# jianfch/stable-ts

Measured on AMD Instinct MI355X. Metric: real-time factor (audio-sec/wall-sec) large-v3 word_timestamps=True, higher is better.
Workload: dtype f16; 1 GPU; large-v3 (random-init, weight recipe BENCH_WEIGHTS = the parity-pinned recipe of tests/test_gpu_f16_depth.py), 10 min synthetic 16 kHz audio per GPU, word_timestamps=True, beam_size=5, 112 decode steps/window, window-parallel batch 20, default regrouping inside the timed pass; mode=transcribe, windows_per_gpu=20, segments=125, words=1670, parallelism=dp1 (windows sharded, no data-path collective)

## Files before the change

include/swx.h:

```cpp
#ifndef SWX_H
#define SWX_H
#include <stdint.h>
#include <stddef.h>

#ifdef __cplusplus
extern "C" {
#endif

#define SWX_F32 0
#define SWX_F16 1

#define SWX_N_SAMPLES 480000
#define SWX_N_FRAMES 3000
#define SWX_N_FFT 400
#define SWX_HOP 160

typedef struct swx_dims {
    int32_t n_mels, n_audio_ctx, n_audio_state, n_audio_head, n_audio_layer;
    int32_t n_vocab, n_text_ctx, n_text_state, n_text_head, n_text_layer;
} swx_dims;

typedef struct swx_model swx_model;

const char *swx_strerror(int code);
// ... 63 lines not shown

size_t swx_qcap_bytes(const swx_model *m, int max_n);
int swx_score_q(swx_model *m, const int32_t *d_tokens, const int32_t *h_n_tok, int max_n, int n_sot, int eot,
                const void *d_xkv, float *d_token_probs, void *d_q, void *stream);
size_t swx_heads_scratch_bytes(const swx_model *m, int max_n);
int swx_heads_dynamic(swx_model *m, const void *d_q, int max_n, int row0, int n_rows, const void *d_xkv, int n_frames,
                      float qk_scale, int count, const double *d_peaks, float *d_qk_sel, int ld_f, void *d_scratch,
                      size_t scratch_bytes, void *stream);
int swx_heads_new(swx_model *m, const void *d_q, int max_n, int n_tok, int row0, int n_out, const void *d_xkv, int n_frames,
                  float qk_scale, int medfilt_width, int topk, float w_colnorm, float w_rownorm, float w_coverage,
                  float *d_neg_matrix, int ld_f, void *d_scratch, size_t scratch_bytes, void *stream);
int swx_weighted_sum(const float *const *h_xs, const float *h_coef, int n_in, float *d_out, int64_t n, void *stream);

size_t swx_qcap_batch_bytes(const swx_model *m, int W, int max_n);
int swx_score_q_batch(swx_model *m, const int32_t *d_tokens, const int32_t *h_n_tok, int W, int max_n, int n_sot, int eot,
                      const void *d_xkv, int xkv_W, float *d_token_probs, void *d_q, void *stream);
size_t swx_heads_batch_scratch_bytes(const swx_model *m, int W, int max_n, int count);
int swx_heads_dynamic_batch(swx_model *m, const void *d_q, int W, int max_n, int n_sot, const int32_t *h_n_tok,
                            const int32_t *h_n_frames, const void *d_xkv, int xkv_W, float qk_scale, int medfilt_width, int count,
                            const double *d_peaks, float *d_neg_matrix, int ld_f, void *d_scratch, size_t scratch_bytes,
                            void *stream);
int swx_heads_new_batch(swx_model *m, const void *d_q, int W, int max_n, int n_sot, const int32_t *h_n_tok,
                        const int32_t *h_n_frames, const void *d_xkv, int xkv_W, float qk_scale, int medfilt_width, int topk,
                        float w_colnorm, float w_rownorm, float w_coverage, float *d_neg_matrix, int ld_f, void *d_scratch,
                        size_t scratch_bytes, void *stream);

int swx_forward_logits(swx_model *m, const int32_t *d_tokens, const int32_t *h_n_tok, int W, int max_n,
                       const void *d_xkv, float *d_logits, void *stream);

int swx_forward_token_ranks(swx_model *m, const int32_t *d_tokens, const int32_t *h_n_tok, int W, int max_n, int n_vocab_used,
                            const void *d_xkv, float *d_prob, int32_t *d_rank, void *stream);

int swx_forward_next_token(swx_model *m, const int32_t *d_tokens, const int32_t *h_n_tok, int W, int max_n, int eot,
                           const int32_t *d_suppress, int n_suppress, const int32_t *d_target,
                           const void *d_xkv, int32_t *d_top , float *d_prob , void *stream);

int swx_detect_language(swx_model *m, const void *d_xkv, int W, int sot, const int32_t *d_lang_tokens, int n_lang,
                        float *d_probs, int32_t *d_best, void *stream);

size_t swx_align_weights_scratch_bytes(int W, int H, int N);
int swx_align_weights(const float *d_qk, int W, int H, int N, int ld_f, const int32_t *h_n_frames, float qk_scale,
                      int medfilt_width, float *d_neg_matrix, void *d_scratch, size_t scratch_bytes, void *stream);

int swx_median_filter(const float *d_x, int64_t rows, int n, int width, float *d_out, void *stream);

int swx_loudness_probe(const float *d_pcm, int64_t pcm_stride, const int32_t *d_nk, const int32_t *d_idx, int n_idx, int W,
                       float *d_out, void *d_scratch, size_t scratch_bytes, void *stream);
size_t swx_loudness_probe_scratch_bytes(int W);

int swx_pcm_edit(const float *d_clean, float *d_probe, int64_t stride, int n_rows, const int32_t *d_ops,
                 const int32_t *d_row_start, int n_ops, void *stream);

typedef struct swx_gate_cfg {
    int32_t n_fft;
    int32_t n_mean;
    float   thresh, slope, prop_decrease;
    int32_t n_grad_freq, n_grad_time;
} swx_gate_cfg;
size_t swx_spectral_gate_scratch_bytes(int rows, const swx_gate_cfg *cfg);
int swx_spectral_gate(const float *d_pcm, int64_t pcm_stride, int rows, int64_t n, const swx_gate_cfg *cfg, float *d_out,
                      int64_t out_stride, void *d_scratch, size_t scratch_bytes, void *stream);
int swx_test_spectral_gate_block(int frames_per_block);

typedef struct swx_flac_info {
    int32_t sample_rate, channels, bits_per_sample, min_block, max_block;
    int64_t total_samples;
    uint8_t md5[16];
} swx_flac_info;
int swx_flac_probe(const uint8_t *h_data, size_t n_bytes, swx_flac_info *info);
int64_t swx_flac_decode(const uint8_t *h_data, size_t n_bytes, int32_t *h_out, int64_t capacity_frames, swx_flac_info *info);

size_t swx_dtw_workspace_bytes(int W, int ld_n, int ld_m);
int swx_dtw(const float *d_x, int W, int ld_n, int ld_m, const int32_t *d_N, const int32_t *d_M,
            int32_t *d_text_idx, int32_t *d_time_idx, int32_t *d_len, void *d_trace_ws, void *stream);

int swx_prof_enable(int on);
int swx_debug_flags(int flags);
int swx_prof_collect(double *out, int n_classes);
int swx_graph_stats(const swx_model *m, int64_t *out);

int swx_test_gemm(int dtype, const void *d_a, int64_t lda, const void *d_w, const float *d_bias, const void *d_res,
                  void *d_c, int64_t ldc, int M, int N, int K, int epilogue, int force_kernel, void *stream);
int swx_test_gemm_plan(int M, int N, int K, int epilogue, int force_kernel, int flags);
int swx_test_dec_gemm(const void *d_a, int64_t lda, const void *d_w, const float *d_gamma, const float *d_beta,
                      const float *d_bias, void *d_c, int64_t ldc, void *d_x, void *d_kcache, void *d_vcache,
                      const int32_t *d_pos0, int n_ctx, int d, int M, int N, int K, int epilogue, void *d_scratch,
                      size_t scratch_bytes, void *stream);
int swx_test_layernorm(int dtype, const void *d_x, const float *d_g, const float *d_b, void *d_y, int rows, int d,
                       void *stream);
int swx_test_attention(int dtype, const void *d_q, int64_t ldq, const void *d_k, const void *d_v, int64_t ldkv,
                       void *d_o, int64_t ldo, int B, int H, int nq, int nk, int force_kernel, int vt_kp, void *stream);

int swx_test_gemm_layout(int dtype, const void *d_a, int64_t lda, const void *d_w, int64_t ldw, const float *d_bias, const void *d_res,
                         const float *d_resf, int res_mod, void *d_c, int64_t ldc, void *d_c2, void *d_p, int64_t p_bs, int p_nkpad,
                         int p_vcol0, int vt_s, int vt_kp, int64_t vt_bs, int vt_zero_pad, int M, int N, int K, int epilogue,
                         int force_kernel, void *stream);
int swx_test_xkv_pack(const void *d_k, const void *d_vt, void *d_packed, int B, int H, int nk, int ldk, int vt_kp, int64_t batch_stride,
                      void *stream);
int swx_test_attention_packed(const void *d_q, int64_t ldq, const void *d_k, const void *d_v, int64_t ldkv, int64_t k_bs, int64_t v_bs,
                              const void *d_packed, void *d_o, int64_t ldo, int B, int H, int nq, int nk, int vt_kp, int force_kernel,
                              const void *d_x, int64_t ldx, int fq_rows, const void *d_wq, const float *d_gamma, const float *d_beta,
                              const float *d_bias, void *d_scratch, size_t scratch_bytes, void *stream);
int swx_test_xattn_plan(int B, int H, int nq, int nk, int vt_kp, int has_packed, int has_fq, int force_kernel, int flags);

int swx_test_self_attn_step(const void *d_q, void *d_kcache, void *d_vcache, const int32_t *d_anc, const int32_t *d_pos0,
                            int R, int H, int n_ctx, int d, int variant, void *d_o, void *stream);

int swx_test_self_attn_multi(const void *d_q, void *d_kcache, void *d_vcache, int R, int H, int n_new, int n_ctx, int d, int mq,
                             void *d_o, void *stream);

int swx_test_self_attn_general(int dtype, const void *d_qkv, int64_t ldqkv, void *d_kcache, void *d_vcache, const int32_t *d_anc,
                               const int32_t *d_pos0, int R, int H, int n_new, int n_ctx, int d, int row_mul, int skip_append,
                               int pos0_all_zero, void *d_o, void *stream);
int swx_test_kcache_index(int k_chunked, int n_ctx, int d, int pos, int h, int chunk);
int swx_test_kcache_relayout(const void *h_src, void *h_dst, int64_t rows, int n_ctx, int d, int elem_bytes, int to_chunked);
int swx_test_dec_gemm_kl(const void *d_a, int64_t lda, const void *d_w, const float *d_gamma, const float *d_beta,
                         const float *d_bias, void *d_c, int64_t ldc, void *d_x, void *d_kcache, void *d_vcache,
                         const int32_t *d_pos0, int n_ctx, int d, int M, int N, int K, int epilogue, int rps, int k_chunked,
                         void *d_scratch, size_t scratch_bytes, void *stream);
int swx_test_self_attn_step_kl(const void *d_q, void *d_kcache, void *d_vcache, const int32_t *d_anc, const int32_t *d_pos0,
                               int R, int H, int n_ctx, int d, int variant, int k_chunked, void *d_o, void *stream);
int swx_test_self_attn_multi_kl(const void *d_q, void *d_kcache, void *d_vcache, int R, int H, int n_new, int n_ctx, int d, int mq,
                                int k_chunked, void *d_o, void *stream);
int swx_test_self_attn_general_kl(int dtype, const void *d_qkv, int64_t ldqkv, void *d_kcache, void *d_vcache, const int32_t *d_anc,
                                  const int32_t *d_pos0, int R, int H, int n_new, int n_ctx, int d, int row_mul, int skip_append,
                                  int pos0_all_zero, int step_variant, int k_chunked, void *d_o, void *stream);
int swx_test_self_attn_plan(int dtype, int R, int H, int n_new, int n_ctx, int row_mul, int skip_append, int step_cached, int pos_bound,
                            int pos0_all_zero, int has_anc, int flags);
int swx_test_dec_plan(int M, int N, int K, int epilogue, int flags);
int swx_test_heads_layout(const swx_model *m, int W, int max_n, int count, int64_t *out);

int swx_test_lane_xor(const uint32_t *d_in, uint32_t *d_out, int n_waves, void *stream);

int swx_test_next_token_reduce(const float *d_logits, int64_t ld, int W, int eot, const int32_t *d_suppress, int n_suppress,
                               const int32_t *d_target, int32_t *d_top, float *d_prob, void *stream);

int swx_test_gelu_pair(uint64_t *d_out, void *stream);

size_t swx_test_decode_script_ws_bytes(const swx_decode_cfg *cfg, int n_vocab, int n_ctx);
int swx_test_decode_script(const swx_decode_cfg *cfg, int n_vocab, int n_ctx, const int32_t *d_init_tokens,
                           const int32_t *d_suppress, const uint8_t *d_ts_mask, const float *d_prefill_logits,
                           const float *d_script, int n_script, int32_t *d_tokens_out, int32_t *d_lens_out, float *d_sumlp_out,
                           float *d_nospeech, int32_t *d_anc_out, int32_t *d_pos0_out, void *d_ws, size_t ws_bytes, void *stream);

int swx_test_sampler_words(uint64_t seed, int64_t row_uid, int step, int id0, int n, uint32_t *d_words, float *d_variates, void *stream);
int swx_test_sampler_buckets(int k0, int n, float *d_variates, void *stream);

#ifdef __cplusplus
}
#endif
#endif
```

stable_ts_amd/_lib.py:

```python
import ctypes
import os
from ctypes import POINTER, Structure, c_char_p, c_float, c_int, c_int32, c_int64, c_size_t, c_uint64, c_void_p

_HERE = os.path.dirname(os.path.abspath(__file__))
LIB_PATH = os.path.join(_HERE, "libswx.so")

SWX_F32 = 0
SWX_F16 = 1


class SwxError(RuntimeError):
    pass


class swx_dims(Structure):
    _fields_ = [(n, c_int32) for n in ("n_mels", "n_audio_ctx", "n_audio_state", "n_audio_head", "n_audio_layer",
                                       "n_vocab", "n_text_ctx", "n_text_state", "n_text_head", "n_text_layer")]


class swx_flac_info(Structure):
    _fields_ = [("sample_rate", c_int32), ("channels", c_int32), ("bits_per_sample", c_int32), ("min_block", c_int32),
                ("max_block", c_int32), ("total_samples", c_int64), ("md5", ctypes.c_uint8 * 16)]


# ... 11 lines not shown
        ("no_speech", c_int32), ("blank_token", c_int32), ("n_suppress", c_int32), ("min_tokens", c_int32),
        ("seed", c_uint64), ("window_uid", POINTER(c_int32)), ("noise", c_void_p),
        ("sample_begins", POINTER(c_int32)), ("sot_indices", POINTER(c_int32)),
    ]


SYMBOLS = {
    "swx_strerror": (c_char_p, [c_int]),
    "swx_version": (c_int, []),
    "swx_model_create": (c_int, [POINTER(swx_dims), c_int, POINTER(c_void_p)]),
    "swx_model_destroy": (None, [c_void_p]),
    "swx_weights_bytes": (c_size_t, [c_void_p]),
    "swx_bind_weights": (c_int, [c_void_p, c_void_p, c_size_t]),
    "swx_share_weights": (c_int, [c_void_p, c_void_p]),
    "swx_load_tensor": (c_int, [c_void_p, c_char_p, c_void_p, c_int64, c_void_p]),
    "swx_weights_complete": (c_int, [c_void_p]),
    "swx_missing_tensor": (c_int, [c_void_p, c_int, c_char_p, c_int]),
    "swx_weights_mark_loaded": (c_int, [c_void_p]),
    "swx_weights_finalize": (c_int, [c_void_p, c_void_p]),
    "swx_set_alignment_heads": (c_int, [c_void_p, POINTER(c_int32), c_int]),
    "swx_num_alignment_heads": (c_int, [c_void_p]),
    "swx_workspace_bytes": (c_size_t, [c_void_p, c_int, c_int]),
    "swx_bind_workspace": (c_int, [c_void_p, c_void_p, c_size_t, c_int, c_int]),
    "swx_log_mel": (c_int, [c_void_p, c_void_p, c_int, c_void_p, c_int, c_void_p]),
    "swx_log_mel_ragged": (c_int, [c_void_p, c_void_p, c_void_p, c_void_p, c_int, c_void_p, c_int, c_void_p]),
    "swx_log_mel_ragged_grouped": (c_int, [c_void_p, c_void_p, c_void_p, c_void_p, c_int, c_void_p, c_int, c_void_p]),
    "swx_encode": (c_int, [c_void_p, c_void_p, c_int, c_void_p, c_void_p]),
    "swx_cross_kv_bytes": (c_size_t, [c_void_p, c_int]),
    "swx_cross_kv": (c_int, [c_void_p, c_void_p, c_int, c_void_p, c_void_p]),
    "swx_decode": (c_int, [c_void_p, POINTER(swx_decode_cfg), c_void_p, c_void_p, c_void_p, c_void_p, c_void_p,
                           c_void_p, c_void_p, c_void_p, c_void_p]),
    "swx_decode_gout": (c_int, [POINTER(swx_decode_cfg)]),
    "swx_score": (c_int, [c_void_p, c_void_p, POINTER(c_int32), c_int, c_int, c_int, c_int, POINTER(c_int32), c_float,
                          c_int, c_void_p, c_void_p, c_void_p, c_void_p]),
    "swx_score_qk": (c_int, [c_void_p, c_void_p, POINTER(c_int32), c_int, c_int, c_int, c_int, c_int, c_int, c_void_p,
                             c_void_p, c_void_p, c_void_p]),
    "swx_qcap_bytes": (c_size_t, [c_void_p, c_int]),
    "swx_score_q": (c_int, [c_void_p, c_void_p, POINTER(c_int32), c_int, c_int, c_int, c_void_p, c_void_p, c_void_p, c_void_p]),
    "swx_heads_scratch_bytes": (c_size_t, [c_void_p, c_int]),
    "swx_heads_dynamic": (c_int, [c_void_p, c_void_p, c_int, c_int, c_int, c_void_p, c_int, c_float, c_int, c_void_p, c_void_p,
                                  c_int, c_void_p, c_size_t, c_void_p]),
    "swx_heads_new": (c_int, [c_void_p, c_void_p, c_int, c_int, c_int, c_int, c_void_p, c_int, c_float, c_int, c_int, c_float,
                              c_float, c_float, c_void_p, c_int, c_void_p, c_size_t, c_void_p]),
    "swx_weighted_sum": (c_int, [c_void_p, c_void_p, c_int, c_void_p, c_int64, c_void_p]),
    "swx_qcap_batch_bytes": (c_size_t, [c_void_p, c_int, c_int]),
    "swx_score_q_batch": (c_int, [c_void_p, c_void_p, POINTER(c_int32), c_int, c_int, c_int, c_int, c_void_p, c_int, c_void_p,
                                  c_void_p, c_void_p]),
    "swx_heads_batch_scratch_bytes": (c_size_t, [c_void_p, c_int, c_int, c_int]),
    "swx_heads_dynamic_batch": (c_int, [c_void_p, c_void_p, c_int, c_int, c_int, POINTER(c_int32), POINTER(c_int32), c_void_p, c_int,
                                        c_float, c_int, c_int, c_void_p, c_void_p, c_int, c_void_p, c_size_t, c_void_p]),
    "swx_heads_new_batch": (c_int, [c_void_p, c_void_p, c_int, c_int, c_int, POINTER(c_int32), POINTER(c_int32), c_void_p, c_int,
                                    c_float, c_int, c_int, c_float, c_float, c_float, c_void_p, c_int, c_void_p, c_size_t, c_void_p]),
    "swx_forward_logits": (c_int, [c_void_p, c_void_p, POINTER(c_int32), c_int, c_int, c_void_p, c_void_p, c_void_p]),
    "swx_forward_token_ranks": (c_int, [c_void_p, c_void_p, POINTER(c_int32), c_int, c_int, c_int, c_void_p, c_void_p, c_void_p,
                                        c_void_p]),
    "swx_forward_next_token": (c_int, [c_void_p, c_void_p, POINTER(c_int32), c_int, c_int, c_int, c_void_p, c_int, c_void_p,
                                       c_void_p, c_void_p, c_void_p, c_void_p]),
    "swx_test_next_token_reduce": (c_int, [c_void_p, c_int64, c_int, c_int, c_void_p, c_int, c_void_p, c_void_p, c_void_p,
                                           c_void_p]),
    "swx_detect_language": (c_int, [c_void_p, c_void_p, c_int, c_int, c_void_p, c_int, c_void_p, c_void_p, c_void_p]),
    "swx_align_weights_scratch_bytes":(c_size_t, [c_int, c_int, c_int]),
    "swx_align_weights": (c_int, [c_void_p, c_int, c_int, c_int, c_int, POINTER(c_int32), c_float, c_int, c_void_p,
                                  c_void_p, c_size_t, c_void_p]),
    "swx_median_filter": (c_int, [c_void_p, c_int64, c_int, c_int, c_void_p, c_void_p]),
    "swx_loudness_probe": (c_int, [c_void_p, c_int64, c_void_p, c_void_p, c_int, c_int, c_void_p, c_void_p, c_size_t, c_void_p]),
    "swx_loudness_probe_scratch_bytes": (c_size_t, [c_int]),
    "swx_pcm_edit": (c_int, [c_void_p, c_void_p, c_int64, c_int, c_void_p, c_void_p, c_int, c_void_p]),
    "swx_spectral_gate_scratch_bytes": (c_size_t, [c_int, POINTER(swx_gate_cfg)]),
    "swx_spectral_gate": (c_int, [c_void_p, c_int64, c_int, c_int64, POINTER(swx_gate_cfg), c_void_p, c_int64, c_void_p, c_size_t,
                                  c_void_p]),
    "swx_test_spectral_gate_block": (c_int, [c_int]),
    "swx_flac_probe": (c_int, [c_void_p, c_size_t, POINTER(swx_flac_info)]),
    "swx_flac_decode": (c_int64, [c_void_p, c_size_t, c_void_p, c_int64, POINTER(swx_flac_info)]),
    "swx_dtw_workspace_bytes": (c_size_t, [c_int, c_int, c_int]),
    "swx_dtw": (c_int, [c_void_p, c_int, c_int, c_int, c_void_p, c_void_p, c_void_p, c_void_p, c_void_p, c_void_p,
                        c_void_p]),
    "swx_prof_enable": (c_int, [c_int]),
    "swx_debug_flags": (c_int, [c_int]),
    "swx_prof_collect": (c_int, [POINTER(ctypes.c_double), c_int]),
    "swx_graph_stats": (c_int, [c_void_p, POINTER(c_int64)]),
    "swx_test_gemm": (c_int, [c_int, c_void_p, c_int64, c_void_p, c_void_p, c_void_p, c_void_p, c_int64, c_int, c_int,
                              c_int, c_int, c_int, c_void_p]),
    "swx_test_gemm_plan": (c_int, [c_int, c_int, c_int, c_int, c_int, c_int]),
    "swx_test_dec_gemm": (c_int, [c_void_p, c_int64, c_void_p, c_void_p, c_void_p, c_void_p, c_void_p, c_int64, c_void_p,
                                  c_void_p, c_void_p, c_void_p, c_int, c_int, c_int, c_int, c_int, c_int, c_void_p, c_size_t,
                                  c_void_p]),
    "swx_test_self_attn_step": (c_int, [c_void_p, c_void_p, c_void_p, c_void_p, c_void_p, c_int, c_int, c_int, c_int, c_int, c_void_p,
                                        c_void_p]),
    "swx_test_self_attn_multi": (c_int, [c_void_p, c_void_p, c_void_p, c_int, c_int, c_int, c_int, c_int, c_int, c_void_p, c_void_p]),
    "swx_test_self_attn_general": (c_int, [c_int, c_void_p, c_int64, c_void_p, c_void_p, c_void_p, c_void_p, c_int, c_int, c_int, c_int,
                                           c_int, c_int, c_int, c_int, c_void_p, c_void_p]),
    "swx_test_kcache_index": (c_int, [c_int] * 6),
    "swx_test_kcache_relayout": (c_int, [c_void_p, c_void_p, c_int64, c_int, c_int, c_int, c_int]),
    "swx_test_dec_gemm_kl": (c_int, [c_void_p, c_int64, c_void_p, c_void_p, c_void_p, c_void_p, c_void_p, c_int64, c_void_p,
                                     c_void_p, c_void_p, c_void_p, c_int, c_int, c_int, c_int, c_int, c_int, c_int, c_int, c_void_p,
                                     c_size_t, c_void_p]),
    "swx_test_self_attn_step_kl": (c_int, [c_void_p, c_void_p, c_void_p, c_void_p, c_void_p, c_int, c_int, c_int, c_int, c_int, c_int,
                                           c_void_p, c_void_p]),
    "swx_test_self_attn_multi_kl": (c_int, [c_void_p, c_void_p, c_void_p, c_int, c_int, c_int, c_int, c_int, c_int, c_int, c_void_p,
                                            c_void_p]),
    "swx_test_self_attn_general_kl": (c_int, [c_int, c_void_p, c_int64, c_void_p, c_void_p, c_void_p, c_void_p, c_int, c_int, c_int,
                                              c_int, c_int, c_int, c_int, c_int, c_int, c_int, c_void_p, c_void_p]),
    "swx_test_self_attn_plan": (c_int, [c_int] * 12),
    "swx_test_dec_plan": (c_int, [c_int, c_int, c_int, c_int, c_int]),
    "swx_test_heads_layout": (c_int, [c_void_p, c_int, c_int, c_int, POINTER(c_int64)]),
    "swx_test_gelu_pair": (c_int, [c_void_p, c_void_p]),
    "swx_test_decode_script_ws_bytes": (c_size_t, [POINTER(swx_decode_cfg), c_int, c_int]),
    "swx_test_decode_script": (c_int, [POINTER(swx_decode_cfg), c_int, c_int, c_void_p, c_void_p, c_void_p, c_void_p, c_void_p,
                                       c_int, c_void_p, c_void_p, c_void_p, c_void_p, c_void_p, c_void_p, c_void_p, c_size_t,
                                       c_void_p]),
    "swx_test_sampler_words": (c_int, [c_uint64, c_int64, c_int, c_int, c_int, c_void_p, c_void_p, c_void_p]),
    "swx_test_sampler_buckets": (c_int, [c_int, c_int, c_void_p, c_void_p]),
    "swx_test_lane_xor": (c_int, [c_void_p, c_void_p, c_int, c_void_p]),
    "swx_test_layernorm": (c_int, [c_int, c_void_p, c_void_p, c_void_p, c_void_p, c_int, c_int, c_void_p]),
    "swx_test_attention": (c_int, [c_int, c_void_p, c_int64, c_void_p, c_void_p, c_int64, c_void_p, c_int64, c_int,
                                   c_int, c_int, c_int, c_int, c_int, c_void_p]),
    "swx_test_gemm_layout": (c_int, [c_int, c_void_p, c_int64, c_void_p, c_int64, c_void_p, c_void_p, c_void_p, c_int, c_void_p,
                                     c_int64, c_void_p, c_void_p, c_int64, c_int, c_int, c_int, c_int, c_int64, c_int, c_int, c_int,
                                     c_int, c_int, c_int, c_void_p]),
    "swx_test_xkv_pack": (c_int, [c_void_p, c_void_p, c_void_p, c_int, c_int, c_int, c_int, c_int, c_int64, c_void_p]),
    "swx_test_attention_packed": (c_int, [c_void_p, c_int64, c_void_p, c_void_p, c_int64, c_int64, c_int64, c_void_p, c_void_p,
                                          c_int64, c_int, c_int, c_int, c_int, c_int, c_int, c_void_p, c_int64, c_int, c_void_p,
                                          c_void_p, c_void_p, c_void_p, c_void_p, c_size_t, c_void_p]),
    "swx_test_xattn_plan": (c_int, [c_int] * 9),
}

_lib = None


def load(build_if_missing: bool = False) -> ctypes.CDLL:
    global _lib
    if _lib is not None:
        return _lib
    if not os.path.exists(LIB_PATH):
        if build_if_missing:
            from .build import build
            build(verbose=False)
        else:
            raise SwxError(f"{LIB_PATH} not found: build it with `python -m stable_ts_amd.build` "
                           f"(hipcc --offload-arch=gfx950). There is no CPU fallback.")
    lib = ctypes.CDLL(LIB_PATH)
    for name, (res, args) in SYMBOLS.items():
        fn = getattr(lib, name)
        fn.restype = res
        fn.argtypes = args
    _lib = lib
    return lib


def check(code: int, what: str = "") -> int:
    if code < 0:
        msg = load().swx_strerror(code).decode()
        raise SwxError(f"{what or 'libswx'} failed: {msg} ({code})")
    return code


def require_gpu():
    import torch
    if not torch.cuda.is_available():
        raise SwxError("stable_ts_amd needs a ROCm GPU (MI355X / gfx950); no CPU path exists in this package")
```

stable_ts_amd/csrc/swx_gemm.hip:

```cpp
#include <cstdlib>
#include <type_traits>
#include <array>
#include <vector>
#include <cstdio>
#include "swx_common.h"
#include "swx_kernels.h"

namespace {

template <typename T>
__device__ __forceinline__ void epilogue_store(const GemmArgs &g, int row, int col, float v)
{
    if (row >= g.M || col >= g.N) return;
    if (g.epi & EPI_BIAS) v += g.bias[col];
    if (g.epi & EPI_GELU) v = gelu_erf(v);
    if (g.epi & EPI_RESF32MOD) v += g.Rf[(size_t)(row % g.res_mod) * g.N + col];
    if (g.epi & EPI_RES) v += to_f32<T>(((const T *)g.R)[(size_t)row * g.ldr + col]);
    if (g.epi & EPI_STORE_VT) {
        const int w = row / g.vt_s, sidx = row - w * g.vt_s;
        ((T *)g.C)[(size_t)w * g.vt_bs + (size_t)col * g.vt_kp + sidx] = from_f32<T>(v);
    } else if (g.epi & EPI_CBATCH) {
        const int w = row / g.vt_s, sidx = row - w * g.vt_s;
        ((T *)g.C)[(size_t)w * g.vt_bs + (size_t)sidx * g.ldc + col] = from_f32<T>(v);
    } else if (g.epi & EPI_OUT_F32) ((float *)g.C)[(size_t)row * g.ldc + col] = v;
// ... 907 lines not shown
    const f16x8 zero8 = (f16x8)(f16)0;

    f16x8 wf[NKS_MAX];
#pragma unroll
    for (int ks = 0; ks < NKS_MAX; ++ks) {
        const f16x8 v = *(const f16x8 *)(wp + (ks < nks ? ks : nks - 1) * 32);
        wf[ks] = (nok && ks < nks) ? v : zero8;
    }

    f32x4 acc[MT];
#pragma unroll
    for (int t = 0; t < MT; ++t) acc[t] = (f32x4){0.f, 0.f, 0.f, 0.f};
    const f16 *ap[MT];
    bool aok[MT];
#pragma unroll
    for (int t = 0; t < MT; ++t) {
        const int m = t * 16 + fr;
        aok[t] = m < g.M;
        ap[t] = A + (size_t)(aok[t] ? m : 0) * g.lda + kb + fk;
    }
    f16x8 af[2][MT];
#pragma unroll
    for (int t = 0; t < MT; ++t) { const f16x8 v = *(const f16x8 *)(ap[t]); af[0][t] = aok[t] ? v : zero8; }
#pragma unroll
    for (int ks = 0; ks < NKS_MAX; ++ks) {
        if (ks < nks) {
            if (ks + 1 < nks) {
#pragma unroll
                for (int t = 0; t < MT; ++t) { const f16x8 v = *(const f16x8 *)(ap[t] + (ks + 1) * 32); af[(ks + 1) & 1][t] = aok[t] ? v : zero8; }
            }
#pragma unroll
            for (int t = 0; t < MT; ++t) acc[t] = __builtin_amdgcn_mfma_f32_16x16x32_f16(af[ks & 1][t], wf[ks], acc[t], 0, 0, 0);
        }
    }

    if (wave > 0) {
#pragma unroll
        for (int t = 0; t < MT; ++t) red[wave - 1][t][lane] = acc[t];
    }
    __syncthreads();
    if (wave == 0) {
        const int col = n0 + (lane & 15), row_l = (lane >> 4) * 4;
#pragma unroll
        for (int t = 0; t < MT; ++t) {
            f32x4 v = acc[t];
#pragma unroll
            for (int w = 0; w < 3; ++w) {
                const f32x4 o = red[w][t][lane];
                v[0] += o[0]; v[1] += o[1]; v[2] += o[2]; v[3] += o[3];
            }
#pragma unroll
            for (int r = 0; r < 4; ++r) epilogue_store<f16>(g, t * 16 + row_l + r, col, v[r]);
        }
    }
}

}

int swx_gemm_plan_f16(int M, int N, int K, int epi, int64_t ldc, int64_t ldr, bool ptr16, int force_kernel, int flags)
{
    if (K % 32 != 0) return -4;
    const bool skinny_ok = M <= 128 && K % 128 == 0 && K / 128 <= 10 && N <= 16384;
    if (force_kernel == 2) return skinny_ok ? SWX_GEMM_SKINNY : -4;
    if (skinny_ok && force_kernel != 1 && force_kernel < 7) return SWX_GEMM_SKINNY;
    const bool glds_ok = K % 64 == 0 && ptr16;
    if (force_kernel >= 7 && !glds_ok) return -4;
    if (force_kernel == 1 || !glds_ok) return SWX_GEMM_TILED_REG;
    const int64_t t128 = (int64_t)cdiv(N, BN) * cdiv(M, BM);
    const bool narrow = force_kernel == 8 || (force_kernel != 9 && N % 64 == 0 && t128 < 224);
    const bool big_ok = !(epi & ~(EPI_BIAS | EPI_GELU | EPI_RES)) && ldc % 8 == 0 && (!(epi & EPI_RES) || ldr % 8 == 0);
    if (force_kernel == 12) return big_ok && K >= 128 ? SWX_GEMM_BIG : -4;
    const int64_t t256 = (int64_t)cdiv(M, BG) * cdiv(N, BG);
    const double fill = (double)t256 / (double)(((t256 + 255) / 256) * 256);
    if (force_kernel == 0 && big_ok && t256 >= 200 && K >= 512 && (fill >= 0.9 || (fill >= 0.75 && K >= 2560)) &&
        !(flags & SWX_FLAG_NO_BIG_TILE))
        return SWX_GEMM_BIG;
    const bool ring_ok = K >= 128;
    if (force_kernel == 10 || force_kernel == 11) return !ring_ok ? -4 : force_kernel == 10 ? SWX_GEMM_RING64 : SWX_GEMM_RING128;
    if (force_kernel == 0 && ring_ok && M > 256 && (narrow || t128 <= 256) && !(flags & SWX_FLAG_NO_RING))
        return narrow ? SWX_GEMM_RING64 : SWX_GEMM_RING128;
    return narrow ? SWX_GEMM_GLDS64 : SWX_GEMM_GLDS128;
}

int swx_gemm(int dtype, const GemmArgs &g, int force_kernel, hipStream_t s)
{
    if (g.M <= 0 || g.N <= 0) return 0;
    if (dtype == SWX_F16) {
        if (g.lda % 8 != 0 || g.ldw % 8 != 0) return -4;
        const bool ptr16 = (uintptr_t)g.A % 16 == 0 && (uintptr_t)g.W % 16 == 0;
        const bool cr16 = (uintptr_t)g.C % 16 == 0 && (!(g.epi & EPI_RES) || (uintptr_t)g.R % 16 == 0);
        const int plan = swx_gemm_plan_f16(g.M, g.N, g.K, g.epi, cr16 ? g.ldc : 1, cr16 ? g.ldr : 1, ptr16, force_kernel, swx_flags());
        if (plan < 0) return plan;
        if (plan == SWX_GEMM_SKINNY) {
            SwxProfScope prof(PC_GEMM_SKINNY, 2.0 * ((double)g.N * g.K + (double)g.M * g.K) + (double)g.M * g.N * ((g.epi & EPI_OUT_F32) ? 4 : 2), s);
            dim3 grid(cdiv(g.N, 16));
            const int mt = cdiv(g.M, 16);
            switch (mt) {
                case 1: hipLaunchKernelGGL(gemm_f16_skinny<1>, grid, dim3(256), 0, s, g); break;
                case 2: hipLaunchKernelGGL(gemm_f16_skinny<2>, grid, dim3(256), 0, s, g); break;
                case 3: hipLaunchKernelGGL(gemm_f16_skinny<3>, grid, dim3(256), 0, s, g); break;
                case 4: hipLaunchKernelGGL(gemm_f16_skinny<4>, grid, dim3(256), 0, s, g); break;
                case 5: hipLaunchKernelGGL(gemm_f16_skinny<5>, grid, dim3(256), 0, s, g); break;
                case 6: hipLaunchKernelGGL(gemm_f16_skinny<6>, grid, dim3(256), 0, s, g); break;
                case 7: hipLaunchKernelGGL(gemm_f16_skinny<7>, grid, dim3(256), 0, s, g); break;
                default: hipLaunchKernelGGL(gemm_f16_skinny<8>, grid, dim3(256), 0, s, g); break;
            }
        } else {
            SwxProfScope prof(PC_GEMM_TILED, 2.0 * (double)g.M * g.N * g.K, s);
            const dim3 grid(cdiv(g.N, BN), cdiv(g.M, BM));
            switch (plan) {
                case SWX_GEMM_BIG: {
                    GemmArgs gb = g;
                    gb.tile_order = (swx_flags() & SWX_FLAG_BIG8_GROUPED) ? 1 : 0;
                    hipLaunchKernelGGL(gemm_f16_big8, dim3(cdiv(g.N, BG), cdiv(g.M, BG)), dim3(512), 2 * B8_BUF, s, gb); break;
                }
                case SWX_GEMM_RING64: launch_ring<64, 3>(g, s); break;
                case SWX_GEMM_RING128: launch_ring<128, 3>(g, s); break;
                case SWX_GEMM_GLDS64: hipLaunchKernelGGL(gemm_f16_glds_64, dim3(cdiv(g.N, 64), grid.y), dim3(256), 0, s, g); break;
                case SWX_GEMM_GLDS128: hipLaunchKernelGGL(gemm_f16_glds_128, grid, dim3(256), 0, s, g); break;
                default: hipLaunchKernelGGL(gemm_f16_tiled, grid, dim3(256), 0, s, g); break;
            }
        }
    } else {
        if (g.K % 16 != 0 || g.lda % 4 != 0 || g.ldw % 4 != 0) return -4;
        SwxProfScope prof(PC_GEMM_TILED, 2.0 * (double)g.M * g.N * g.K, s);
        if (g.M <= BM && g.N >= 256 && g.K % 64 == 0 && force_kernel != 8) {
            if (g.N >= 2560) hipLaunchKernelGGL((gemm_f32_rows64<2>), dim3(cdiv(g.N, 32), cdiv(g.M, 64)), dim3(256), 0, s, g);
            else hipLaunchKernelGGL((gemm_f32_rows64<1>), dim3(cdiv(g.N, 16), cdiv(g.M, 64)), dim3(256), 0, s, g);
        } else if (g.M <= BM && g.N >= 256) {
            if (g.N >= 2560) hipLaunchKernelGGL((gemm_f32_tiled<64, 32, 4>), dim3(cdiv(g.N, 32), cdiv(g.M, 64)), dim3(256), 0, s, g);
            else hipLaunchKernelGGL((gemm_f32_tiled<64, 16, 4>), dim3(cdiv(g.N, 16), cdiv(g.M, 64)), dim3(256), 0, s, g);
        } else {
            hipLaunchKernelGGL((gemm_f32_tiled<128, 128, 4>), dim3(cdiv(g.N, BN), cdiv(g.M, BM)), dim3(256), 0, s, g);
        }
    }
    SWX_CHECK_LAUNCH();
    return 0;
}
```

stable_ts_amd/csrc/swx_kernels.h:

```cpp
#pragma once
#include <hip/hip_runtime.h>
#include <stdint.h>
#include "../../include/swx.h"

#define EPI_BIAS 1
#define EPI_GELU 2
#define EPI_RES 4
#define EPI_OUT_F32 8
#define EPI_RESF32MOD 16
#define EPI_CBATCH 64
#define EPI_STORE_VT 32
#define EPI_KV 128

#define EPI_QKV_VT 256

struct GemmArgs {
    const void *A; int64_t lda;
    const void *W; int64_t ldw;
    const float *bias;
    const void *R; int64_t ldr;
    const float *Rf; int res_mod;
    void *C; int64_t ldc;
    void *C2;
    void *P; int64_t p_bs;
    int p_nkpad, p_vcol0;
    int M, N, K;
    int epi;
    int vt_s, vt_kp; int64_t vt_bs;
    int vt_zero_pad;
    int tile_order;
};
int swx_gemm(int dtype, const GemmArgs &g, int force_kernel, hipStream_t s);
enum { SWX_GEMM_TILED_REG = 0, SWX_GEMM_SKINNY = 1, SWX_GEMM_GLDS128 = 2, SWX_GEMM_GLDS64 = 3, SWX_GEMM_RING64 = 4, SWX_GEMM_RING128 = 5,
       SWX_GEMM_BIG = 6 };
int swx_gemm_plan_f16(int M, int N, int K, int epi, int64_t ldc, int64_t ldr, bool ptr16, int force_kernel, int flags);

#define SWX_FLAG_TABLE(X) \
    X(NO_FAST_STEP, 0)         \
    X(KCACHE_CHUNKED, 1)       \
    X(SELFATTN_NO_DEEP, 2)     \
    X(DEC_NO_W1, 4)            \
    X(TALL_NO_W8, 5)           \
    X(FLASH_NO_QB1, 6)         \
    X(XKV_PACK_SEPARATE, 7)    \
    X(SELFATTN_NO_MQ, 8)       \
    X(XQ_FULL_TILE, 9)         \
    X(DEC_W1_FULL_TILE, 10)    \
    X(NO_PACKED_XKV, 11)       \
    X(SELECT_MEM, 13)          \
    X(NO_GRAPH, 14)            \
    X(NO_PREFETCH, 15)         \
    X(NO_RING, 16)             \
    X(NO_BIG_TILE, 17)         \
    X(SCORE_TILED, 18)         \
    X(NO_TALL, 19)             \
    X(NO_FUSED_XQ, 20)         \
    X(TICKET, 21)              \
    X(BIG8_GROUPED, 22)        \
    X(XKV_TWO_LAUNCHES, 23)    \
    X(LOUDNESS_ONE_WG, 24)     \
    X(XATTN_R5, 25)            \
    X(FLASH_PIPELINED, 26)     \
    X(SELFATTN_WG5, 27)        \
    X(QKV_SEPARATE_VT, 28)
#define SWX_FLAG_DEFINE(name, bit) constexpr int SWX_FLAG_##name = 1 << (bit);
SWX_FLAG_TABLE(SWX_FLAG_DEFINE)
#undef SWX_FLAG_DEFINE
#define SWX_FLAG_IN_RANGE(name, bit) && (bit) >= 0 && (bit) <= 30
#define SWX_FLAG_OR(name, bit) | (int64_t(1) << (bit))
#define SWX_FLAG_SUM(name, bit) + (int64_t(1) << (bit))
static_assert(true SWX_FLAG_TABLE(SWX_FLAG_IN_RANGE), "SWX_FLAG_TABLE: a bit index outside 0..30");
static_assert((int64_t(0) SWX_FLAG_TABLE(SWX_FLAG_OR)) == (int64_t(0) SWX_FLAG_TABLE(SWX_FLAG_SUM)), "SWX_FLAG_TABLE: two switches share a bit");
#undef SWX_FLAG_IN_RANGE
#undef SWX_FLAG_OR
#undef SWX_FLAG_SUM
#define SWX_DEFAULT_FLAGS 0
int swx_flags();

struct KLayout { int sp, sh, sc; };
__host__ __device__ inline KLayout swx_klayout(int chunked, int n_ctx, int d)
{
    return chunked ? KLayout{8, 64 * n_ctx, 8 * n_ctx} : KLayout{d, 64, 8};
}
__host__ __device__ inline int swx_kidx(const KLayout &L, int pos, int h, int chunk) { return h * L.sh + chunk * L.sc + pos * L.sp; }

#define DEC_LN 1
#define DEC_GELU 2
#define DEC_RES 4
#define DEC_QKV 8
#define DEC_SLAB 16
#define DEC_TICKET 32
struct DecPrefetch {
    const void *base;
    int lines;
};
DecPrefetch swx_dec_prefetch_of(const void *packed_w, int M, int N, int K, int epi);

struct DecGemmArgs {
    const _Float16 *A; int64_t lda;
    const _Float16 *W; int64_t ldw;
    int M, N, K;
    int epi;
    const float *c2;
    const float *c1;
    _Float16 *C; int64_t ldc;
    _Float16 *X; int64_t ldx;
    float *slabs;
    int *ticket;
    _Float16 *kcache, *vcache; const int32_t *pos0; int n_ctx, d;
    KLayout kl;
    int rps;
    int row_mul;
    int ks2, kslice, n_rg; int64_t slab_stride;
    int tall;
    int tps;
    DecPrefetch pf;
    int w1_full_tile;
};
#define SWX_DEC_TICKETS 4096
int swx_dec_plan(int M, int N, int K, int epi, int *mt, int *ks2);
size_t swx_dec_slab_floats(int M, int N, int K);
int swx_gemm_dec(DecGemmArgs g, hipStream_t s);
enum SwxDecKernel { SWX_DEC_K_W4 = 0,
                    SWX_DEC_K_W1 = 1,
                    SWX_DEC_K_TALL4 = 2,
                    SWX_DEC_K_TALL8 = 3 };
int swx_dec_kernel_plan(int M, int N, int K, int epi, int tall, bool ticket_ok, int flags, int *mt, int *ks2, bool *ticket);
int swx_fold_ln(const void *W, const float *gamma, const float *beta, const float *bias, void *Wf, float *c1, float *c2,
                int N, int K, hipStream_t s);

enum SwxProfClass { PC_GEMM_TILED = 0, PC_GEMM_SKINNY = 1, PC_ATTN_FLASH = 2, PC_ATTN_ROWWISE = 3, PC_SELF_ATTN = 4,
// ... 108 lines not shown
```

stable_ts_amd/csrc/swx_testhooks.hip:

```cpp
#include <cstring>
#include "swx_model.h"

__global__ __launch_bounds__(64) void lane_xor_check_kernel(const uint32_t *__restrict__ in, uint32_t *__restrict__ out)
{
    const int lane = threadIdx.x;
    const uint32_t x = in[blockIdx.x * 64 + lane];
    uint32_t *o = out + (size_t)blockIdx.x * 13 * 64 + lane;
    o[0 * 64] = lane_xor_u32<32>(x, lane); o[1 * 64] = lane_xor_u32<16>(x, lane); o[2 * 64] = lane_xor_u32<8>(x, lane);
    o[3 * 64] = lane_xor_u32<4>(x, lane);  o[4 * 64] = lane_xor_u32<2>(x, lane);  o[5 * 64] = lane_xor_u32<1>(x, lane);
    o[6 * 64] = (uint32_t)__shfl_xor((int)x, 32, 64); o[7 * 64] = (uint32_t)__shfl_xor((int)x, 16, 64);
    o[8 * 64] = (uint32_t)__shfl_xor((int)x, 8, 64);  o[9 * 64] = (uint32_t)__shfl_xor((int)x, 4, 64);
    o[10 * 64] = (uint32_t)__shfl_xor((int)x, 2, 64); o[11 * 64] = (uint32_t)__shfl_xor((int)x, 1, 64);
    double v = (double)__uint_as_float(x);
    double ref = v;
#pragma unroll
    for (int off = 32; off > 0; off >>= 1) ref += __shfl_xor(ref, off, 64);
    const double got = wave_sum_d(v);
    unsigned ok = (__double_as_longlong(got) == __double_as_longlong(ref)) ? 1u : 0u;
    const float f = (float)(int)(x >> 9) * 1.1920929e-7f - 0.37f;
    ok |= (__float_as_uint(lane_xor16_max(f)) == __float_as_uint(fmaxf(f, __shfl_xor(f, 16, 64)))) ? 2u : 0u;
    ok |= (__float_as_uint(lane_xor32_max(f)) == __float_as_uint(fmaxf(f, __shfl_xor(f, 32, 64)))) ? 4u : 0u;
    ok |= (__float_as_uint(lane_xor16_add(f)) == __float_as_uint(f + __shfl_xor(f, 16, 64))) ? 8u : 0u;
    ok |= (__float_as_uint(lane_xor32_add(f)) == __float_as_uint(f + __shfl_xor(f, 32, 64))) ? 16u : 0u;
    float wm = f, ws = f;
#pragma unroll
    for (int off = 32; off > 0; off >>= 1) { wm = fmaxf(wm, __shfl_xor(wm, off, 64)); ws += __shfl_xor(ws, off, 64); }
    ok |= (__float_as_uint(wave_max(f)) == __float_as_uint(wm)) ? 32u : 0u;
    ok |= (__float_as_uint(wave_sum(f)) == __float_as_uint(ws)) ? 64u : 0u;
    o[12 * 64] = ok;
}

__global__ __launch_bounds__(256) void gelu_pair_check_kernel(unsigned long long *__restrict__ out)
{
    const unsigned base = (blockIdx.x * 256u + threadIdx.x) * 32u;
    unsigned bad = 0, nan_bits = 0, first = 0xffffffffu;
#pragma unroll 4
    for (unsigned j = 0; j < 32; j += 2) {
        const unsigned u0 = base + j, u1 = base + j + 1;
        const f32x2 x = {__uint_as_float(u0), __uint_as_float(u1)};
        const f32x2 got = gelu_erf2(x);
        const float r0 = gelu_erf(x[0]), r1 = gelu_erf(x[1]);
        const unsigned g0 = __float_as_uint(got[0]), g1 = __float_as_uint(got[1]), e0 = __float_as_uint(r0), e1 = __float_as_uint(r1);
        if (g0 != e0) { if (r0 != r0 && got[0] != got[0]) ++nan_bits; else { ++bad; first = first < u0 ? first : u0; } }
        if (g1 != e1) { if (r1 != r1 && got[1] != got[1]) ++nan_bits; else { ++bad; first = first < u1 ? first : u1; } }
    }
    if (bad) { atomicAdd(out, (unsigned long long)bad); atomicMin(out + 1, (unsigned long long)first); }
    if (nan_bits) atomicAdd(out + 2, (unsigned long long)nan_bits);
}

__global__ __launch_bounds__(256) void sampler_words_kernel(uint64_t seed, unsigned row_uid, unsigned step, unsigned id0, unsigned n,
                                                            uint32_t *__restrict__ words, float *__restrict__ variates)
{
    const unsigned i = blockIdx.x * 256u + threadIdx.x;
    if (i >= n) return;
    words[i] = sampler_word(seed, row_uid, step, id0 + i);
    variates[i] = gumbel(seed, row_uid, step, id0 + i);
}

__global__ __launch_bounds__(256) void sampler_buckets_kernel(unsigned k0, unsigned n, float *__restrict__ variates)
{
    const unsigned i = blockIdx.x * 256u + threadIdx.x;
    if (i >= n) return;
    variates[i] = sampler_variate((k0 + i) << 8);
}

extern "C" {

int swx_test_sampler_words(uint64_t seed, int64_t row_uid, int step, int id0, int n, uint32_t *d_words, float *d_variates, void *stream)
{
    if (!d_words || !d_variates || n <= 0 || step < 0 || id0 < 0 || (int64_t)id0 + n > (int64_t)1 << 31) return -1;
    hipLaunchKernelGGL(sampler_words_kernel, dim3(((unsigned)n + 255u) / 256u), dim3(256), 0, S(stream), seed, (unsigned)(uint64_t)row_uid,
                       (unsigned)step, (unsigned)id0, (unsigned)n, d_words, d_variates);
    SWX_CHECK_LAUNCH();
    return 0;
}

int swx_test_sampler_buckets(int k0, int n, float *d_variates, void *stream)
{
    if (!d_variates || n <= 0 || k0 < 0 || (int64_t)k0 + n > (int64_t)1 << 24) return -1;
    hipLaunchKernelGGL(sampler_buckets_kernel, dim3(((unsigned)n + 255u) / 256u), dim3(256), 0, S(stream), (unsigned)k0, (unsigned)n, d_variates);
    SWX_CHECK_LAUNCH();
    return 0;
}

int swx_test_gemm(int dtype, const void *d_a, int64_t lda, const void *d_w, const float *d_bias, const void *d_res,
                  void *d_c, int64_t ldc, int M, int N, int K, int epilogue, int force_kernel, void *stream)
{
    GemmArgs g = swx_gemm_args(d_a, lda, d_w, K, d_bias, d_c, ldc, M, N, K, epilogue);
    g.R = d_res; g.ldr = ldc;
    return swx_gemm(dtype, g, force_kernel, S(stream));
}

int swx_test_gemm_plan(int M, int N, int K, int epilogue, int force_kernel, int flags)
{
    return swx_gemm_plan_f16(M, N, K, epilogue, N, N, true, force_kernel, flags);
}

int swx_test_dec_gemm(const void *d_a, int64_t lda, const void *d_w, const float *d_gamma, const float *d_beta, const float *d_bias,
                      void *d_c, int64_t ldc, void *d_x, void *d_kcache, void *d_vcache, const int32_t *d_pos0, int n_ctx, int d,
                      int M, int N, int K, int epilogue, void *d_scratch, size_t scratch_bytes, void *stream)
{
    return swx_test_dec_gemm_kl(d_a, lda, d_w, d_gamma, d_beta, d_bias, d_c, ldc, d_x, d_kcache, d_vcache, d_pos0, n_ctx, d, M, N, K, epilogue,
                                0, 0, d_scratch, scratch_bytes, stream);
}

int swx_test_dec_gemm_kl(const void *d_a, int64_t lda, const void *d_w, const float *d_gamma, const float *d_beta, const float *d_bias,
                         void *d_c, int64_t ldc, void *d_x, void *d_kcache, void *d_vcache, const int32_t *d_pos0, int n_ctx, int d,
                         int M, int N, int K, int epilogue, int rps, int k_chunked, void *d_scratch, size_t scratch_bytes, void *stream)
{
    if (k_chunked && (epilogue & DEC_QKV) && (n_ctx <= 0 || d <= 0 || d % 64)) return -2;
    hipStream_t s = S(stream);
    unsigned char *p = (unsigned char *)d_scratch;
    const size_t slab_b = align_up(swx_dec_slab_floats(M, N, K) * 4 + 256);
    const size_t need = align_up((size_t)N * K * 2) + 2 * align_up((size_t)N * 4) + slab_b + (size_t)SWX_DEC_TICKETS * 4;
    if (scratch_bytes < need) return -8;
    f16 *wf = (f16 *)p; p += align_up((size_t)N * K * 2);
    float *c1 = (float *)p; p += align_up((size_t)N * 4);
    float *c2 = (float *)p; p += align_up((size_t)N * 4);
    float *slabs = (float *)p; p += slab_b;
    int *ticket = (int *)p;
    if (!(epilogue & 128)) { hipError_t e = hipMemsetAsync(ticket, 0, (size_t)SWX_DEC_TICKETS * 4, s); if (e != hipSuccess) return -100 - (int)e; }
    DecGemmArgs g{};
    g.A = (const f16 *)d_a; g.lda = lda; g.M = M; g.N = N; g.K = K; g.epi = epilogue; g.ldw = K;
    g.C = (f16 *)d_c; g.ldc = ldc; g.X = (f16 *)d_x; g.ldx = ldc; g.slabs = slabs; g.ticket = ticket;
    g.kcache = (f16 *)d_kcache; g.vcache = (f16 *)d_vcache; g.pos0 = d_pos0; g.n_ctx = n_ctx; g.d = d;
    g.epi = epilogue & 31;
    g.tall = (epilogue & 64) ? 1 : 0;
    g.rps = (epilogue & 64) && (epilogue & DEC_QKV) ? 7 : 0;
    if (rps > 0 && (epilogue & DEC_QKV)) g.rps = rps;
    g.kl = swx_klayout(k_chunked ? 1 : 0, n_ctx, d);
    if ((epilogue & DEC_LN) && (epilogue & 32)) {
        g.W = (const f16 *)d_w; g.c1 = d_gamma; g.c2 = d_beta;
    } else if (epilogue & DEC_LN) {
        SWX_TRY(swx_fold_ln(d_w, d_gamma, d_beta, d_bias, wf, c1, c2, N, K, s));
        g.W = wf; g.c1 = c1; g.c2 = c2;
    } else if (epilogue & 32) {
        g.W = (const f16 *)d_w; g.c2 = d_bias;
    } else {
        SWX_TRY(swx_fold_ln(d_w, nullptr, nullptr, nullptr, wf, nullptr, nullptr, N, K, s));
        g.W = wf; g.c2 = d_bias;
    }
    return swx_gemm_dec(g, s);
}

int swx_test_self_attn_step(const void *d_q, void *d_kcache, void *d_vcache, const int32_t *d_anc, const int32_t *d_pos0,
                            int R, int H, int n_ctx, int d, int variant, void *d_o, void *stream)
{
    return swx_test_self_attn_step_kl(d_q, d_kcache, d_vcache, d_anc, d_pos0, R, H, n_ctx, d, variant, 0, d_o, stream);
}

int swx_test_self_attn_step_kl(const void *d_q, void *d_kcache, void *d_vcache, const int32_t *d_anc, const int32_t *d_pos0,
                               int R, int H, int n_ctx, int d, int variant, int k_chunked, void *d_o, void *stream)
{
    if (d != 64 * H) return -2;
    SelfAttnArgs sa{};
    sa.kl = swx_klayout(k_chunked ? 1 : 0, n_ctx, d);
    sa.qkv = d_q; sa.ldqkv = d; sa.kcache = d_kcache; sa.vcache = d_vcache; sa.anc = (int32_t *)d_anc; sa.pos0 = d_pos0;
    sa.o = d_o; sa.ldo = d; sa.R = R; sa.n_new = 1; sa.H = H; sa.n_ctx = n_ctx; sa.d = d; sa.skip_append = 1;
    sa.step_cached = variant < 2 ? 1 : 0;
    sa.pos_bound = variant == 0 ? 128 : 0;
    return swx_self_attention(SWX_F16, sa, 1, S(stream));
}

int swx_test_self_attn_multi(const void *d_q, void *d_kcache, void *d_vcache, int R, int H, int n_new, int n_ctx, int d, int mq,
                             void *d_o, void *stream)
{
    return swx_test_self_attn_multi_kl(d_q, d_kcache, d_vcache, R, H, n_new, n_ctx, d, mq, 0, d_o, stream);
}

int swx_test_self_attn_multi_kl(const void *d_q, void *d_kcache, void *d_vcache, int R, int H, int n_new, int n_ctx, int d, int mq,
                                int k_chunked, void *d_o, void *stream)
{
    static int32_t *d_zeros = nullptr;
    static int zeros_n = 0;
    if (R <= 0 || n_new <= 0 || n_new > n_ctx) return -2;
    if (zeros_n < R) {
        if (d_zeros) (void)hipFree(d_zeros);
        zeros_n = 0; d_zeros = nullptr;
// ... 205 lines not shown
```

Baseline: 1473 x real time.

## Split f16 GEMMs into big-tile body and small-tile tail to fix wave quantization

Adds a cost-model-driven split for f16 GEMMs. The rows that fill whole big8 waves across the 256 CUs go to the big-tile kernel, and the leftover rows go to a ring or GLDS kernel. The aim is to avoid a mostly empty final round of 256x256 tiles when M does not divide evenly. The split costs an extra kernel launch and relies on hard-coded per-round timing constants. It can be disabled with a new flag.

```diff
diff --git a/include/swx.h b/include/swx.h
--- a/include/swx.h
+++ b/include/swx.h
@@ -169,6 +169,10 @@
 int swx_test_gemm(int dtype, const void *d_a, int64_t lda, const void *d_w, const float *d_bias, const void *d_res,
                   void *d_c, int64_t ldc, int M, int N, int K, int epilogue, int force_kernel, void *stream);
 int swx_test_gemm_plan(int M, int N, int K, int epilogue, int force_kernel, int flags);
+int swx_test_gemm_split_plan(int M, int N, int K, int epilogue, int flags, int n_cu, int *tail_kernel);
+int swx_test_gemm_tail_plan(int M, int N, int K, int force_kernel, int flags);
+int swx_test_gemm_split(const void *d_a, int64_t lda, const void *d_w, const float *d_bias, const void *d_res, void *d_c, int64_t ldc,
+                        int M, int N, int K, int epilogue, int body_rows, int tail_force, void *stream);
 int swx_test_dec_gemm(const void *d_a, int64_t lda, const void *d_w, const float *d_gamma, const float *d_beta,
                       const float *d_bias, void *d_c, int64_t ldc, void *d_x, void *d_kcache, void *d_vcache,
                       const int32_t *d_pos0, int n_ctx, int d, int M, int N, int K, int epilogue, void *d_scratch,
diff --git a/stable_ts_amd/_lib.py b/stable_ts_amd/_lib.py
--- a/stable_ts_amd/_lib.py
+++ b/stable_ts_amd/_lib.py
@@ -117,6 +117,10 @@
     "swx_test_gemm": (c_int, [c_int, c_void_p, c_int64, c_void_p, c_void_p, c_void_p, c_void_p, c_int64, c_int, c_int,
                               c_int, c_int, c_int, c_void_p]),
     "swx_test_gemm_plan": (c_int, [c_int, c_int, c_int, c_int, c_int, c_int]),
+    "swx_test_gemm_split_plan": (c_int, [c_int, c_int, c_int, c_int, c_int, c_int, POINTER(c_int)]),
+    "swx_test_gemm_tail_plan": (c_int, [c_int, c_int, c_int, c_int, c_int]),
+    "swx_test_gemm_split": (c_int, [c_void_p, c_int64, c_void_p, c_void_p, c_void_p, c_void_p, c_int64, c_int, c_int, c_int, c_int,
+                                    c_int, c_int, c_void_p]),
     "swx_test_dec_gemm": (c_int, [c_void_p, c_int64, c_void_p, c_void_p, c_void_p, c_void_p, c_void_p, c_int64, c_void_p,
                                   c_void_p, c_void_p, c_void_p, c_int, c_int, c_int, c_int, c_int, c_int, c_void_p, c_size_t,
                                   c_void_p]),
diff --git a/stable_ts_amd/csrc/swx_gemm.hip b/stable_ts_amd/csrc/swx_gemm.hip
--- a/stable_ts_amd/csrc/swx_gemm.hip
+++ b/stable_ts_amd/csrc/swx_gemm.hip
@@ -1013,6 +1013,103 @@
     return narrow ? SWX_GEMM_GLDS64 : SWX_GEMM_GLDS128;
 }
 
+int swx_gemm_tail_plan_f16(int M, int N, int K, int force_kernel, int flags, int n_cu)
+{
+    if (M <= 0 || K % 64 != 0 || K < 128) return -4;
+    switch (force_kernel) {
+        case 0: break;
+        case 8: return SWX_GEMM_GLDS64;
+        case 9: return SWX_GEMM_GLDS128;
+        case 10: return SWX_GEMM_RING64;
+        case 11: return SWX_GEMM_RING128;
+        default: return -4;
+    }
+    const int64_t t128 = (int64_t)cdiv(N, BN) * cdiv(M, BM);
+    const bool narrow = N % 64 == 0 && t128 < 224;
+    if (M > 256 && (narrow || t128 <= 256) && !(flags & SWX_FLAG_NO_RING)) return narrow ? SWX_GEMM_RING64 : SWX_GEMM_RING128;
+    return narrow || (N % 64 == 0 && 2 * t128 <= 3 * (int64_t)n_cu) ? SWX_GEMM_GLDS64 : SWX_GEMM_GLDS128;
+}
+
+constexpr double SPLIT_FILL = 0.95;
+constexpr double SPLIT_MARGIN_US = 10.0;
+constexpr double B8_ROUND_US0 = 11.0, B8_ROUND_US_PER_KT = 1.55, B8_ROUND_US_GELU = 9.0;
+constexpr double SMALL_US0 = 12.9, SMALL_US_PER_KT = 0.62;
+static double b8_round_us(int K, int epi) { return B8_ROUND_US0 + B8_ROUND_US_PER_KT * (K / 64) + ((epi & EPI_GELU) ? B8_ROUND_US_GELU : 0.0); }
+static double small_us(int64_t t128, int K, int n_cu)
+{
+    const double per_cu = (double)t128 / n_cu;
+    return SMALL_US0 + SMALL_US_PER_KT * (K / 64) * (per_cu > 1.0 ? per_cu : 1.0);
+}
+
+int swx_gemm_split_f16(int M, int N, int K, int epi, int64_t ldc, int64_t ldr, bool ptr16, int flags, int n_cu, int *body_rows)
+{
+    *body_rows = 0;
+    if (flags & (SWX_FLAG_NO_GEMM_SPLIT | SWX_FLAG_NO_BIG_TILE)) return -1;
+    if (n_cu <= 0 || M <= BG || K % 64 != 0 || K < 512 || !ptr16) return -1;
+    if ((epi & ~(EPI_BIAS | EPI_GELU | EPI_RES)) || ldc % 8 != 0 || ((epi & EPI_RES) && ldr % 8 != 0)) return -1;
+    const int whole = swx_gemm_plan_f16(M, N, K, epi, ldc, ldr, ptr16, 0, flags);
+    if (whole < 0 || whole == SWX_GEMM_SKINNY || whole == SWX_GEMM_TILED_REG) return -1;
+    const int tn = cdiv(N, BG);
+    int r = (M - 1) / BG;
+    for (; r > 0; --r) {
+        const int64_t t = (int64_t)r * tn, rounds = (t + n_cu - 1) / n_cu;
+        if ((double)t >= SPLIT_FILL * (double)(rounds * n_cu)) break;
+    }
+    if (r <= 0) return -1;
+    const int body = r * BG, tail = M - body;
+    const int tail_plan = swx_gemm_tail_plan_f16(tail, N, K, 0, flags, n_cu);
+    if (tail_plan < 0) return -1;
+    const int64_t t256 = (int64_t)cdiv(M, BG) * tn, t128 = (int64_t)cdiv(M, BM) * cdiv(N, BN);
+    const double unsplit = whole == SWX_GEMM_BIG ? (double)((t256 + n_cu - 1) / n_cu) * b8_round_us(K, epi) : small_us(t128, K, n_cu);
+    const double split = (double)(((int64_t)r * tn + n_cu - 1) / n_cu) * b8_round_us(K, epi) + small_us((int64_t)cdiv(tail, BM) * cdiv(N, BN), K, n_cu);
+    if (split + SPLIT_MARGIN_US >= unsplit) return -1;
+    *body_rows = body;
+    return tail_plan;
+}
+
+static void launch_f16_tiled_plan(int plan, const GemmArgs &g, hipStream_t s)
+{
+    const dim3 grid(cdiv(g.N, BN), cdiv(g.M, BM));
+    switch (plan) {
+        case SWX_GEMM_BIG: {
+            GemmArgs gb = g;
+            gb.tile_order = (swx_flags() & SWX_FLAG_BIG8_GROUPED) ? 1 : 0;
+            hipLaunchKernelGGL(gemm_f16_big8, dim3(cdiv(g.N, BG), cdiv(g.M, BG)), dim3(512), 2 * B8_BUF, s, gb); break;
+        }
+        case SWX_GEMM_RING64: launch_ring<64, 3>(g, s); break;
+        case SWX_GEMM_RING128: launch_ring<128, 3>(g, s); break;
+        case SWX_GEMM_GLDS64: hipLaunchKernelGGL(gemm_f16_glds_64, dim3(cdiv(g.N, 64), grid.y), dim3(256), 0, s, g); break;
+        case SWX_GEMM_GLDS128: hipLaunchKernelGGL(gemm_f16_glds_128, grid, dim3(256), 0, s, g); break;
+        default: hipLaunchKernelGGL(gemm_f16_tiled, grid, dim3(256), 0, s, g); break;
+    }
+}
+
+static void launch_f16_split(const GemmArgs &g, int body_rows, int tail_plan, hipStream_t s)
+{
+    GemmArgs gb = g;
+    gb.M = body_rows;
+    launch_f16_tiled_plan(SWX_GEMM_BIG, gb, s);
+    GemmArgs gt = g;
+    gt.M = g.M - body_rows;
+    gt.A = (const f16 *)g.A + (size_t)body_rows * g.lda;
+    gt.C = (f16 *)g.C + (size_t)body_rows * g.ldc;
+    if (g.R) gt.R = (const f16 *)g.R + (size_t)body_rows * g.ldr;
+    launch_f16_tiled_plan(tail_plan, gt, s);
+}
+
+int swx_gemm_split_forced(const GemmArgs &g, int body_rows, int tail_force, hipStream_t s)
+{
+    if (body_rows <= 0 || body_rows % BG != 0 || body_rows >= g.M || g.lda % 8 != 0 || g.ldw % 8 != 0) return -4;
+    const bool ptr16 = (uintptr_t)g.A % 16 == 0 && (uintptr_t)g.W % 16 == 0;
+    const bool cr16 = (uintptr_t)g.C % 16 == 0 && (!(g.epi & EPI_RES) || (uintptr_t)g.R % 16 == 0);
+    if (swx_gemm_plan_f16(body_rows, g.N, g.K, g.epi, cr16 ? g.ldc : 1, cr16 ? g.ldr : 1, ptr16, 12, 0) != SWX_GEMM_BIG) return -4;
+    const int tail_plan = swx_gemm_tail_plan_f16(g.M - body_rows, g.N, g.K, tail_force, swx_flags(), SWX_GEMM_CUS);
+    if (tail_plan < 0) return tail_plan;
+    launch_f16_split(g, body_rows, tail_plan, s);
+    SWX_CHECK_LAUNCH();
+    return 0;
+}
+
 int swx_gemm(int dtype, const GemmArgs &g, int force_kernel, hipStream_t s)
 {
     if (g.M <= 0 || g.N <= 0) return 0;
@@ -1038,19 +1135,11 @@
             }
         } else {
             SwxProfScope prof(PC_GEMM_TILED, 2.0 * (double)g.M * g.N * g.K, s);
-            const dim3 grid(cdiv(g.N, BN), cdiv(g.M, BM));
-            switch (plan) {
-                case SWX_GEMM_BIG: {
-                    GemmArgs gb = g;
-                    gb.tile_order = (swx_flags() & SWX_FLAG_BIG8_GROUPED) ? 1 : 0;
-                    hipLaunchKernelGGL(gemm_f16_big8, dim3(cdiv(g.N, BG), cdiv(g.M, BG)), dim3(512), 2 * B8_BUF, s, gb); break;
-                }
-                case SWX_GEMM_RING64: launch_ring<64, 3>(g, s); break;
-                case SWX_GEMM_RING128: launch_ring<128, 3>(g, s); break;
-                case SWX_GEMM_GLDS64: hipLaunchKernelGGL(gemm_f16_glds_64, dim3(cdiv(g.N, 64), grid.y), dim3(256), 0, s, g); break;
-                case SWX_GEMM_GLDS128: hipLaunchKernelGGL(gemm_f16_glds_128, grid, dim3(256), 0, s, g); break;
-                default: hipLaunchKernelGGL(gemm_f16_tiled, grid, dim3(256), 0, s, g); break;
-            }
+            int body_rows = 0;
+            const int tail_plan = force_kernel == 0 ? swx_gemm_split_f16(g.M, g.N, g.K, g.epi, cr16 ? g.ldc : 1, cr16 ? g.ldr : 1, ptr16,
+                                                                         swx_flags(), SWX_GEMM_CUS, &body_rows) : -1;
+            if (body_rows > 0) launch_f16_split(g, body_rows, tail_plan, s);
+            else launch_f16_tiled_plan(plan, g, s);
         }
     } else {
         if (g.K % 16 != 0 || g.lda % 4 != 0 || g.ldw % 4 != 0) return -4;
diff --git a/stable_ts_amd/csrc/swx_kernels.h b/stable_ts_amd/csrc/swx_kernels.h
--- a/stable_ts_amd/csrc/swx_kernels.h
+++ b/stable_ts_amd/csrc/swx_kernels.h
@@ -34,6 +34,10 @@
 enum { SWX_GEMM_TILED_REG = 0, SWX_GEMM_SKINNY = 1, SWX_GEMM_GLDS128 = 2, SWX_GEMM_GLDS64 = 3, SWX_GEMM_RING64 = 4, SWX_GEMM_RING128 = 5,
        SWX_GEMM_BIG = 6 };
 int swx_gemm_plan_f16(int M, int N, int K, int epi, int64_t ldc, int64_t ldr, bool ptr16, int force_kernel, int flags);
+constexpr int SWX_GEMM_CUS = 256;
+int swx_gemm_split_f16(int M, int N, int K, int epi, int64_t ldc, int64_t ldr, bool ptr16, int flags, int n_cu, int *body_rows);
+int swx_gemm_tail_plan_f16(int M, int N, int K, int force_kernel, int flags, int n_cu);
+int swx_gemm_split_forced(const GemmArgs &g, int body_rows, int tail_force, hipStream_t s);
 
 #define SWX_FLAG_TABLE(X) \
     X(NO_FAST_STEP, 0)         \
@@ -47,6 +51,7 @@
     X(XQ_FULL_TILE, 9)         \
     X(DEC_W1_FULL_TILE, 10)    \
     X(NO_PACKED_XKV, 11)       \
+    X(NO_GEMM_SPLIT, 12)       \
     X(SELECT_MEM, 13)          \
     X(NO_GRAPH, 14)            \
     X(NO_PREFETCH, 15)         \
diff --git a/stable_ts_amd/csrc/swx_testhooks.hip b/stable_ts_amd/csrc/swx_testhooks.hip
--- a/stable_ts_amd/csrc/swx_testhooks.hip
+++ b/stable_ts_amd/csrc/swx_testhooks.hip
@@ -94,6 +94,24 @@
 int swx_test_gemm_plan(int M, int N, int K, int epilogue, int force_kernel, int flags)
 {
     return swx_gemm_plan_f16(M, N, K, epilogue, N, N, true, force_kernel, flags);
+}
+
+int swx_test_gemm_split_plan(int M, int N, int K, int epilogue, int flags, int n_cu, int *tail_kernel)
+{
+    int body_rows = 0;
+    const int tail = swx_gemm_split_f16(M, N, K, epilogue, N, N, true, flags, n_cu, &body_rows);
+    if (tail_kernel) *tail_kernel = tail;
+    return body_rows;
+}
+
+int swx_test_gemm_tail_plan(int M, int N, int K, int force_kernel, int flags) { return swx_gemm_tail_plan_f16(M, N, K, force_kernel, flags, SWX_GEMM_CUS); }
+
+int swx_test_gemm_split(const void *d_a, int64_t lda, const void *d_w, const float *d_bias, const void *d_res, void *d_c, int64_t ldc,
+                        int M, int N, int K, int epilogue, int body_rows, int tail_force, void *stream)
+{
+    GemmArgs g = swx_gemm_args(d_a, lda, d_w, K, d_bias, d_c, ldc, M, N, K, epilogue);
+    g.R = d_res; g.ldr = ldc;
+    return swx_gemm_split_forced(g, body_rows, tail_force, S(stream));
 }
 
 int swx_test_dec_gemm(const void *d_a, int64_t lda, const void *d_w, const float *d_gamma, const float *d_beta, const float *d_bias,
```

Result: no change. 1477 x real time (median of 4 runs) (+0.2%).
